# thelovelab/DESeq2

Measured on AMD Instinct MI355X. Metric: genes/sec for DESeq() disp+beta+Wald fit, 50k x 500 x p=4 (throughput of steps pipelined two deep; one call at a time: one_call_at_a_time), higher is better.
Workload: dtype f64; 1 GPU; BASELINE configs[2]: 50k genes x 500 samples, ~batch+condition (p=4), Wald; 50000 non-zero genes in total, sharded over 1 GPU(s) in the contiguous ranges of R/parallel.R:10; inputs resident in HBM in R layout (int32 counts, f64 nf matrix; the fused chain reads the size factors as the m-vector the matrix was built from); genes_total=50000, genes_this_gpu=50000, samples=500, p=4, test=Wald, parallelism=gene-shard x1, chain=fused device-driven (dsq_deseq_dev), steps_overlap=step k enqueued while step k-1's results are copied and post-processed

## Files before the change

deseq2_amd/csrc/aux.hip:

```cpp
#include "dsq_internal.hpp"
#include "dsq_math.hpp"
#include "dsq_wave.hpp"

namespace dsq {

static constexpr int kAuxBatch = 4;

static inline int aux_grid_fwd(int n) {
    int blocks = (n + 3) / 4;
    int cap = device_cu_count() * 8;
    return blocks < cap ? (blocks < 1 ? 1 : blocks) : cap;
}

static constexpr int kTileS = 256;
__host__ __device__ static inline bool aux_tiled(int m, int p) { return (size_t)m * p >= 8192 && p <= 24; }

template <int P, bool USE_W, bool TILED>
__global__ void __launch_bounds__(256) prefit_kernel(PrefitKernelParams kp) {
    extern __shared__ __attribute__((aligned(16))) double tile[];
    const int lane = threadIdx.x & 63;
    const int wave = threadIdx.x >> 6;
    const int waves = blockDim.x >> 6;
    const int m = kp.m;
    double rr[P][P];
// ... 114 lines not shown
#pragma unroll
        for (int c = P - 1; c >= 0; c--) {
            double v = tu[P + c];
#pragma unroll
            for (int k = c + 1; k < P; k++) v = __builtin_fma(-rr[c][k], b[k], v);
            b[c] = v / rr[c][c];
        }
        if (lane == 0 && active) {
            kp.baseMean[g] = mean;
            kp.baseVar[g] = av / (double)(m - 1);
            kp.allZero[g] = (a2[1] == 0.0) ? 1 : 0;
            kp.roughDisp[g] = __builtin_fmax(ae / (double)(m - P), 0.0);
#pragma unroll
            for (int c = 0; c < P; c++) kp.beta_init[(size_t)g + (size_t)kp.n * c] = b[c];
        }
    }
}

template <int P, bool TILED>
__global__ void __launch_bounds__(256) linear_mu_kernel(PrefitKernelParams kp, double mu_floor, double *mu_out) {
    extern __shared__ __attribute__((aligned(16))) double tile[];
    const int lane = threadIdx.x & 63;
    const int wave = threadIdx.x >> 6;
    const int waves = blockDim.x >> 6;
    const int m = kp.m;
    const int nwork = DSQ_NWORK(kp);
    for (int wbase = blockIdx.x * waves; wbase < nwork; wbase += gridDim.x * waves) {
        const int wi = wbase + wave;
        const bool active = wi < nwork;
        if (!TILED && !active) break;
// ... 488 lines not shown
```

deseq2_amd/csrc/ctx.hip:

```cpp
#include "../../include/deseq2_mi355x.h"
#include "dsq_internal.hpp"

#include <cstdarg>
#include <cstdio>
#include <cstdlib>
#include <cstring>
#include <map>
#include <memory>
#include <mutex>
#include <vector>

namespace dsq {

thread_local char g_err[512] = "";
std::mutex g_mu;

int capi_fail(int code, const char *fmt, ...) {
    va_list ap;
    va_start(ap, fmt);
    vsnprintf(g_err, sizeof g_err, fmt, ap);
    va_end(ap);
    return code;
}

int env_int(const char *name, int dflt) {
    const char *v = getenv(name);
    return (v && *v) ? atoi(v) : dflt;
}

const Tuning &tuning() {
    static Tuning t = {env_int("DSQ_BETA_WAVES", 4), env_int("DSQ_BETA_STAGE", -1), env_int("DSQ_BETA_BPC", 0),
                       env_int("DSQ_BETA_LDS_KB", 160),
                       env_int("DSQ_DISP_WAVES", 4), env_int("DSQ_DISP_STAGE", -1), env_int("DSQ_DISP_BPC", 0),
                       env_int("DSQ_DISP_LDS_KB", 160), env_int("DSQ_ABLATE", 0), env_int("DSQ_FORCE_ITERS", 0),
                       env_int("DSQ_DISP_XLDS", 1), env_int("DSQ_BETA_XLDS", 1), env_int("DSQ_DYNAMIC", 1),
                       env_int("DSQ_BETA_CELLS", 1), env_int("DSQ_DISP_CELL_MINP", DSQ_DISP_CELL_MINP),
                       env_int("DSQ_OVERLAP", 1), env_int("DSQ_LPT", 1),
                       env_int("DSQ_LPT_MAXN", 16384), env_int("DSQ_LPT_KEY1", 1), env_int("DSQ_LPT_KEYD", 1), env_int("DSQ_LPT_KEYM", 2),
                       env_int("DSQ_LPT_KEY2", 1), env_int("DSQ_OUTLIER_FIRST", 1)};
    return t;
}

int device_cu_count() {
    static int cached[kMaxDevices];
    int dev = 0;
    if (hipGetDevice(&dev) != hipSuccess || dev < 0 || dev >= kMaxDevices) return 256;
    if (cached[dev] == 0) {
        int v = 0;
        if (hipDeviceGetAttribute(&v, hipDeviceAttributeMultiprocessorCount, dev) != hipSuccess || v <= 0) v = 256;
        cached[dev] = v;
    }
    return cached[dev];
}

// ... 202 lines not shown
```

deseq2_amd/csrc/dsq_internal.hpp:

```cpp
#pragma once
#include <hip/hip_runtime.h>
#include <stdint.h>
#include <functional>
#include <mutex>
#include <string.h>

namespace dsq {

struct DispKernelParams {
    int n, m, p;
    long ld;
    const int32_t *y;
    const double *mu_hat;
    const double *weights;
    const double *x;
    const double *log_alpha_in;
    const double *prior_mean;
    double prior_sigmasq, min_log_alpha, kappa_0, tol, weightThreshold;
    int maxit, usePrior, useWeights, useCR;
    double *log_alpha;
    int32_t *iter, *iter_accept;
    double *last_change, *initial_lp, *initial_dlp, *last_lp, *last_dlp, *last_d2lp;
    const double *grid;
    int ngrid;
// ... 43 lines not shown
};

struct PrefitKernelParams {
    int n, m, p;
    long ld;
    const int32_t *y;
    const double *nf;
    int nf_is_vector;
    const double *weights;
    int useWeights;
    const double *q, *a, *r;
    double *baseMean, *baseVar, *roughDisp, *beta_init;
    int32_t *allZero;
    const int32_t *rows;
    const int32_t *n_dev;
};

struct LogLikeKernelParams {
    int n, m;
    long ld;
    const int32_t *y;
    const double *mu;
    const double *disp;
    const double *weights;
    int useWeights;
    double *loglike;
    const int32_t *rows;
    const int32_t *n_dev;
    const int32_t *skip;
    const double *kconst;
// ... 61 lines not shown
struct ReplaceKernelParams {
    int n, m;
    long ld;
    const int32_t *y;
    const double *nf;
    int nf_is_vector;
    const double *cooks;
    double cutoff, trim;
    const int32_t *replaceable;
    int sortcap;
    int32_t *newCounts, *replace;
    const int32_t *rows;
    const int32_t *n_dev;
    const int32_t *skip;
    int rows_few, beside;
};

struct SizeFactorKernelParams {
    int n, m;
    const void *y;
    long y_si, y_sj;
    const double *nm;
    long nm_si, nm_sj;
    const double *geoMeans;
    const int32_t *control;
    int type;
    int stabilize;
    double *sf;
    double *lgm_out;
    double *nf_out;
// ... 171 lines not shown
    int beta_waves, beta_stage, beta_bpc, beta_lds_kb;
    int disp_waves, disp_stage, disp_bpc, disp_lds_kb;
    int ablate, force_iters;
    int disp_xlds, beta_xlds;
    int dynamic;
    int beta_cells;
    int disp_cell_minp;
    int overlap;
    int lpt;
    int lpt_maxn;
    int lpt_key1;
    int lpt_keyd;
    int lpt_keym;
    int lpt_key2;
    int outlier_first;
};
const Tuning &tuning();

hipError_t launch_transpose_r_to_gm_f64(const double *src, double *dst, int n, int m, long ld, hipStream_t st);
hipError_t launch_transpose_r_to_gm_i32(const int32_t *src, int32_t *dst, int n, int m, long ld, hipStream_t st);
hipError_t launch_counts_f64_to_gm_i32(const double *src, int32_t *dst, int n, int m, long ld, int32_t *bad, hipStream_t st);
hipError_t launch_transpose_gm_to_r_f64(const double *src, double *dst, int n, int m, long ld, hipStream_t st);
hipError_t launch_transpose_gm_to_r_i32(const int32_t *src, int32_t *dst, int n, int m, long ld, hipStream_t st);
hipError_t launch_test_math(int op, const double *a, const double *b, const double *c, double *out, long n, hipStream_t st);

constexpr int kMaxDevices = 64;
int device_cu_count();
#define DSQ_CACHE_PER_DEVICE(a, b)                                                        \
    do {                                                                                  \
        static thread_local int cache_dev_ = -1;                                          \
// ... 48 lines not shown
```

deseq2_amd/csrc/fit_disp.hip:

```cpp
#ifndef DSQ_DISP_WIDE_MIN
#define DSQ_DISP_WIDE_MIN 11
#endif
#define DSQ_WIDE_MIN DSQ_DISP_WIDE_MIN
#include "dsq_internal.hpp"
#include <cstdio>
#include <cstdlib>
#include "dsq_math.hpp"
#include "dsq_rows.hpp"
#include "dsq_wave.hpp"

namespace dsq {

#ifndef DSQ_DISP_LANE_MIN
#define DSQ_DISP_LANE_MIN 4
#endif
#ifndef DSQ_DISP_TRIP_BATCH
#define DSQ_DISP_TRIP_BATCH 4
#endif
#include "../../include/dsq_arith_spec.h"
#ifndef DSQ_DISP_ROWPASS_MIN
#define DSQ_DISP_ROWPASS_MIN DSQ_SPEC_SERIAL_GRAM_MINP
#endif
typedef double DsqMat1[1][DSQ_P][DSQ_P];
typedef double DsqMat2[2][DSQ_P][DSQ_P];
// ... 845 lines not shown
#define DSQ_DISP_MINW_LONG (DSQ_P <= 10 ? 3 : 1)
#endif
template <bool USE_W, bool STAGE, int MODE>
__host__ __device__ constexpr bool disp_global_dv() { return !STAGE && !USE_W && MODE != 2; }
__host__ __device__ inline size_t disp_hist_doubles(int p, int m) { return (p >= 4 && m >= 256 && m <= 2560) ? ((size_t)m + 1) / 2 : 0; }

template <int P, bool USE_W, bool STAGE, int MODE>
__global__ void __launch_bounds__(256, (disp_global_dv<USE_W, STAGE, MODE>() ? DSQ_DISP_MINW_LONG : DSQ_DISP_MINW)) fit_disp_kernel(DispKernelParams kp) {
    extern __shared__ __attribute__((aligned(16))) double smem[];
    const int lane = threadIdx.x & 63;
    const int wave = threadIdx.x >> 6;
    const int waves = blockDim.x >> 6;
    const int m = kp.m;
    const int nwork = DSQ_NWORK(kp);
    if (blockIdx.x * waves >= nwork) return;

    const double *xs = smem;
    const bool serial_gram = disp_serial_gram(P, kp.ncell, m);
    const size_t slab_d = disp_global_dv<USE_W, STAGE, MODE>() ? disp_hist_doubles(P, m) + (serial_gram ? (size_t)3 * m : 0)
                                                               : disp_slab_doubles<USE_W>(m, STAGE, serial_gram);
    const size_t xoff = (STAGE && kp.xlds) ? (size_t)P * m : 0;
    double *slab = smem + xoff + (size_t)wave * slab_d;
    double *arena = smem + xoff + (size_t)waves * slab_d + (size_t)wave * disp_arena_doubles(P, kp.ncell);
    int32_t *cstart_s = reinterpret_cast<int32_t *>(smem + xoff + (size_t)waves * (slab_d + disp_arena_doubles(P, kp.ncell)));
    int32_t *cperm_s = cstart_s + DSQ_CMAX + 2;
    int32_t *crep_s = cperm_s;
    uint8_t *cid_s = reinterpret_cast<uint8_t *>(crep_s + DSQ_CMAX);
    const int C = kp.ncell;
    const bool sorted = disp_sorted<USE_W>(STAGE, C);
    if (C > 0) {
// ... 327 lines not shown
```

deseq2_amd/csrc/outlier.hip:

```cpp
#include "dsq_internal.hpp"
#include "dsq_math.hpp"
#include "dsq_wave.hpp"
#include <type_traits>

namespace dsq {

DSQ_DEV void wave_sort(double *b, int n2, int lane) {
    wave_lds_sync();
    for (int k = 2; k <= n2; k <<= 1) {
        for (int j = k >> 1; j > 0; j >>= 1) {
            for (int t = lane; t < (n2 >> 1); t += 64) {
                int lo = ((t & ~(j - 1)) << 1) | (t & (j - 1));
                int hi = lo | j;
                bool asc = (lo & k) == 0;
                double a = b[lo], c = b[hi];
                if ((a > c) == asc) { b[lo] = c; b[hi] = a; }
            }
            wave_lds_sync();
        }
    }
}

DSQ_DEV void wave_merge_bitonic(double *b, int n2, int lane) {
    wave_lds_sync();
// ... 192 lines not shown
        any = __any(any);
        int32_t *og = kp.newCounts + (size_t)g * kp.ld;
        if (!any) {
            int32_t yb[kOutlierBatch];
            sweep_batched<kOutlierBatch>(m, lane, [&](int j, int b) { yb[b] = yg[j]; }, [&](int j, int b) { og[j] = yb[b]; });
        } else {
            wave_lds_sync();
            for (int k = lane; k < n2; k += 64) buf[k] = k < m ? (double)yg[k] / nfg[k] : inf;
            wave_sort(buf, n2, lane);
            const double tbm = trimmed_mean_sorted(buf, m, kp.trim, lane);
            for (int j = lane; j < m; j += 64) {
                int rep = (int)(tbm * nfg[j]);
                og[j] = (ckg[j] > kp.cutoff && kp.replaceable[j]) ? rep : yg[j];
            }
        }
        if (lane == 0) kp.replace[g] = any ? 1 : 0;
    }
}

static int outlier_waves(size_t doubles_per_wave) {
    const size_t cap = 160 * 1024;
    int w = 4;
    while (w > 0 && (size_t)w * doubles_per_wave * 8 > cap) w >>= 1;
    return w;
}

template <typename KP, typename F>
static hipError_t launch_outlier(F fn, const KP &kp, size_t doubles_per_wave, hipStream_t st, bool *ok) {
    int waves = outlier_waves(doubles_per_wave);
    *ok = waves > 0;
    if (!*ok) return hipSuccess;
// ... 41 lines not shown
```

deseq2_amd/csrc/pipeline.hip:

```cpp
#include "capi.hpp"
#include "dsq_math.hpp"
#include "dsq_wave.hpp"

#include <algorithm>
#include <cstdio>
#include <cstdlib>
#include <cstring>
#include <vector>

namespace dsq {

DSQ_DEV double np_min(double a, double b) { return (a != a || b != b) ? a + b : (a < b ? a : b); }
DSQ_DEV double np_max(double a, double b) { return (a != a || b != b) ? a + b : (a > b ? a : b); }

struct Rows {
    const int32_t *rows;
    const int32_t *n_dev;
    int n;
};
DSQ_DEV int rows_count(const Rows &r) { return r.n_dev ? *r.n_dev : r.n; }
DSQ_DEV int rows_gene(const Rows &r, int i) { return r.rows ? r.rows[i] : i; }

__global__ void __launch_bounds__(1024) compact_kernel(int mode, int n, int32_t *allZero, const int32_t *force_zero,
                                                       const double *mean_in, const double *disp_in, double thresh,
// ... 101 lines not shown
    int32_t *grid_flag, *grid_rows, *grid_count;
    const double *scalars;
    double *dispFit, *log_dfit, *la_init, *dispMAP, *dispersion;
    const double *dispFit_in;
    int32_t *dispIter, *dispOutlier;
    const double *beta_nat, *beta_var, *beta_iter, *logLike;
    double *beta, *betaSE, *stat, *pvalue, *betaIter_out;
    int32_t *betaConv, *optim_flag, *optim_count;
    int32_t *optim_rows;
    int wald;
    const double *beta_init;
    double *opt_start;
    const int32_t *opt_conv;
    LptKey lpt;
    int *lpt_bins;
};

__global__ void alpha_init_kernel(RuleParams q) {
    const int i = blockIdx.x * blockDim.x + threadIdx.x;
    const bool on = i < rows_count(q.rw);
    const int g = on ? rows_gene(q.rw, i) : 0;
    if (on) {
        const double bm = q.baseMean[g], bv = q.baseVar[g];
        const double xim = q.xim_dev ? *q.xim_dev : q.xim;
        const double mom = (bv - xim * bm) / (bm * bm);
        double a = np_min(q.roughDisp[g], mom);
        a = np_min(np_max(q.minDisp, a), q.maxDisp);
        q.alpha_init[g] = a;
        q.la0[g] = dlog(a);
    }
// ... 4 lines not shown
    const int i = blockIdx.x * blockDim.x + threadIdx.x;
    if (i >= rows_count(q.rw)) return;
    const int g = rows_gene(q.rw, i);
    double d = np_min(dexp(q.la_out[g]), q.maxDisp);
    const double ilp = q.initial_lp[g];
    if (q.last_lp[g] < ilp + __builtin_fabs(ilp) / 1e6) d = q.alpha_init[g];
    const int it = q.iter[g];
    q.dispGeneIter[g] = it;
    const bool conv = (it < q.maxit) && !(it == 1);
    const bool refit = !conv && (d > q.minDisp * 10.0);
    q.dge[g] = d;
    q.grid_flag[g] = refit ? 1 : 0;
    if (refit) q.grid_rows[atomicAdd(q.grid_count, 1)] = g;
}

__global__ void gene_est_final_kernel(RuleParams q) {
    const int i = blockIdx.x * blockDim.x + threadIdx.x;
    if (i >= rows_count(q.rw)) return;
    const int g = rows_gene(q.rw, i);
    double d = q.dge[g];
    if (q.grid_flag[g]) d = dexp(q.la_grid[g]);
    q.dge[g] = np_min(np_max(d, q.minDisp), q.maxDisp);
}

__global__ void map_init_kernel(RuleParams q) {
    const int i = blockIdx.x * blockDim.x + threadIdx.x;
    const bool on = i < rows_count(q.rw);
    const int g = on ? rows_gene(q.rw, i) : 0;
    if (on) {
        const double fit = q.dispFit_in ? q.dispFit_in[g] : q.scalars[DSQ_SC_COEF0] + q.scalars[DSQ_SC_COEF1] / q.baseMean[g];
        const double d = q.dge[g];
        double init = (d > 0.1 * fit) ? d : fit;
        if (init != init) init = fit;
        q.dispFit[g] = fit;
        q.log_dfit[g] = dlog(fit);
        q.la_init[g] = dlog(init);
    }
    if (q.lpt.kind != LPT_NONE) lpt_block_hist(on ? lpt_bin(q.lpt, g) : -1, q.lpt_bins);
}

__global__ void map_post_kernel(RuleParams q) {
    const int i = blockIdx.x * blockDim.x + threadIdx.x;
    if (i >= rows_count(q.rw)) return;
    const int g = rows_gene(q.rw, i);
// ... 66 lines not shown
__global__ void optim_post_kernel(RuleParams q) {
    const int cnt = rows_count(q.rw);
    for (int i = blockIdx.x * blockDim.x + threadIdx.x; i < cnt; i += gridDim.x * blockDim.x) {
        const int g = rows_gene(q.rw, i);
        if (q.betaConv && q.opt_conv[g]) q.betaConv[g] = 1;
        if (q.wald && q.stat) {
            for (int c = 0; c < q.p; c++) {
                const double z = q.beta[(size_t)g + (size_t)q.n * c] / q.betaSE[(size_t)g + (size_t)q.n * c];
                q.stat[(size_t)g + (size_t)q.n * c] = z;
                q.pvalue[(size_t)g + (size_t)q.n * c] = dpnorm_upper2(z);
            }
        }
    }
}

__global__ void list_kernel(Rows rw, const int32_t *flag, int want, int32_t *rows_out, int32_t *count) {
    const int i = blockIdx.x * blockDim.x + threadIdx.x;
    if (i >= rows_count(rw)) return;
    const int g = rows_gene(rw, i);
    if ((flag[g] != 0) == (want != 0)) rows_out[atomicAdd(count, 1)] = g;
}

__global__ void cand_list_kernel(Rows rw, const int32_t *bound_flag, const int32_t *optim_flag, int32_t *flag_out, int32_t *rows_out,
                                 int32_t *count) {
    const int i = blockIdx.x * blockDim.x + threadIdx.x;
    if (i >= rows_count(rw)) return;
    const int g = rows_gene(rw, i);
    const int f = (bound_flag[g] != 0 || optim_flag[g] != 0) ? 1 : 0;
    flag_out[g] = f;
    if (f) rows_out[atomicAdd(count, 1)] = g;
}

struct NaRowsParams {
    Rows rw;
    int n, p;
    const int32_t *allZero, *n_refit;
    double *beta, *betaSE, *stat, *pvalue, *betaIter, *logLike, *logLikeReduced, *maxCooks;
    int32_t *betaConv;
};
__global__ void na_rows_kernel(NaRowsParams q) {
    const int i = blockIdx.x * blockDim.x + threadIdx.x;
    if (i >= rows_count(q.rw) || *q.n_refit <= 0) return;
    const int g = rows_gene(q.rw, i);
    if (!q.allZero[g]) return;
    const double nan = dnan();
    for (int c = 0; c < q.p; c++) {
        q.beta[(size_t)g + (size_t)q.n * c] = nan;
        q.betaSE[(size_t)g + (size_t)q.n * c] = nan;
        if (q.stat) { q.stat[(size_t)g + (size_t)q.n * c] = nan; q.pvalue[(size_t)g + (size_t)q.n * c] = nan; }
    }
    q.betaIter[g] = nan; q.logLike[g] = nan; q.maxCooks[g] = nan;
    if (q.logLikeReduced) q.logLikeReduced[g] = nan;
    q.betaConv[g] = -1;
}

__global__ void __launch_bounds__(256) na_assay_rows_kernel(int n, int m, long ld, const int32_t *allZero, double *a0, double *a1,
                                                            int32_t *zero_p = nullptr, int zero_n = 0) {
    if (blockIdx.x == 0 && (int)threadIdx.x < zero_n) zero_p[threadIdx.x] = 0;
    const int lane = threadIdx.x & 63;
    const int g = blockIdx.x * blockDim.x + threadIdx.x;
    unsigned long long todo = __ballot(g < n && allZero[g] != 0);
    const int base = g - lane;
    const double nan = dnan();
    while (todo) {
        const int l = __builtin_ctzll(todo);
        todo &= todo - 1;
        const size_t row = (size_t)(base + l) * ld;
        for (int j = lane; j < m; j += 64) {
            if (a0) a0[row + j] = nan;
            if (a1) a1[row + j] = nan;
        }
    }
}

__global__ void __launch_bounds__(256) masked_max_kernel(Rows rw, int m, long ld, const double *cooks, const int32_t *use,
                                                         const int32_t *zero, int all_replaceable, int valid,
                                                         const int32_t *n_refit, double *maxCooks) {
    if (*n_refit <= 0) return;
    const int lane = threadIdx.x & 63, wave = threadIdx.x >> 6, waves = blockDim.x >> 6;
    const int nw = rows_count(rw);
    for (int wi = blockIdx.x * waves + wave; wi < nw; wi += gridDim.x * waves) {
        const int g = rows_gene(rw, wi);
        if (all_replaceable || !valid) {
            if (lane == 0) maxCooks[g] = dnan();
            continue;
        }
        const double *ck = cooks + (size_t)g * ld;
        double mx = -__builtin_inf();
        int isnan_ = 0;
        for (int j = lane; j < m; j += 64) {
            if (!use[j]) continue;
            double v = zero[j] ? 0.0 : ck[j];
            if (v != v) isnan_ = 1;
// ... 102 lines not shown
    int red_ncell;
    int32_t *cells_dev;
    void *trend_ws, *sel_ws;
    int pkp, pmax;
    int next_counter;
    const int32_t *cell_perm, *cell_start;
    int ncell;
    const char *tag;
    double t_tol, t_minmu, ge_floor;
    int t_maxit, t_useQR;
    hipStream_t side;
    hipEvent_t ev_fork, ev_join;
    bool overlap, forked, ll_pending;
    LogLikeKernelParams ll;
    bool outlier_first, cand_ready, ll_event;
    int any3, maxcell, all_replaceable;
};

enum { CNT_NZ = DSQ_ST_N_NONZERO, CNT_GRID1 = DSQ_ST_N_GRID_GENEEST, CNT_TREND = DSQ_ST_N_TREND, CNT_GRID2 = DSQ_ST_N_GRID_MAP,
       CNT_OPT1 = DSQ_ST_N_OPTIM_GENEEST, CNT_OPT2 = DSQ_ST_N_OPTIM_TEST, CNT_REP = DSQ_ST_N_REPLACE, CNT_REFIT = DSQ_ST_N_REFIT,
       CNT_GRID1R = DSQ_ST_N_GRID_GENEEST_REFIT, CNT_GRID2R = DSQ_ST_N_GRID_MAP_REFIT, CNT_OPT1R = DSQ_ST_N_OPTIM_GENEEST_REFIT,
       CNT_OPT2R = DSQ_ST_N_OPTIM_TEST_REFIT, CNT_OPT3 = 14, CNT_OPT3R = 15, CNT_N = DSQ_ST_COUNT };
static_assert(DSQ_ST_N_OPTIM_TEST_REFIT < 14 && DSQ_ST_COUNT == 16, "status block layout");

static int *next_work_counter(Pipe &P) {
    int *c = P.work_counters + (P.next_counter % 60);
    P.next_counter++;
    return c;
}

static inline dim3 ew_grid(int n) { return dim3((unsigned)((n + 255) / 256 > 0 ? (n + 255) / 256 : 1)); }

static inline int rows_few(const Pipe &P, const Rows &rw) {
    return (rw.rows && rw.rows != P.rows_nz && rw.rows != P.rows_lpt && rw.rows != P.rows_rev) ? 1 : 0;
}

template <class KP>
static KP fit_head(const Pipe &P, const Rows &rw, const int32_t *y, const double *weights) {
    KP kp;
    memset(&kp, 0, sizeof kp);
    kp.n = P.n; kp.m = P.m; kp.ld = P.ld;
    kp.y = y; kp.nf = P.a->nf; kp.nf_is_vector = P.a->nf_is_vector;
    kp.weights = P.a->useWeights ? weights : nullptr; kp.useWeights = kp.weights ? 1 : 0;
    kp.rows = rw.rows; kp.n_dev = rw.n_dev;
    return kp;
}

static RuleParams rule_params(const Pipe &P, const Rows &rw) {
    RuleParams q;
// ... 108 lines not shown
                                       const double *r, double *beta_init) {
    PrefitKernelParams kp = fit_head<PrefitKernelParams>(P, rw, y, nullptr);
    kp.p = p; kp.q = q; kp.a = xr; kp.r = r;
    kp.baseMean = P.cnum; kp.baseVar = P.cden; kp.roughDisp = P.dev; kp.allZero = P.opt_conv; kp.beta_init = beta_init;
    return kp;
}
static LogLikeKernelParams loglike_params(const Pipe &P, const Rows &rw, const int32_t *y, const double *mu, double *out) {
    LogLikeKernelParams lk;
    memset(&lk, 0, sizeof lk);
    lk.n = P.n; lk.m = P.m; lk.ld = P.ld; lk.y = y; lk.mu = mu; lk.disp = P.o->dispersion;
    lk.weights = P.a->useWeights ? P.a->weights_norm : nullptr; lk.useWeights = P.a->useWeights ? 1 : 0;
    lk.loglike = out; lk.rows = rw.rows; lk.n_dev = rw.n_dev; lk.kconst = P.kconst;
    return lk;
}

static int launch_prefit_rows(Pipe &P, const Rows &rw, const int32_t *y) {
    PrefitKernelParams kp = prefit_params(P, rw, y, P.a->weights_raw);
    kp.r = P.a->r;
    kp.baseMean = P.o->baseMean; kp.baseVar = P.o->baseVar; kp.roughDisp = P.roughDisp; kp.beta_init = P.beta_init;
    kp.allZero = P.o->allZero;
    bool ok = false;
    capi_prof_begin(rw.rows ? "prefit_moments:refit" : "prefit_moments", P.n, P.st);
    DSQ_HIP(launch_prefit(kp, P.st, &ok));
    capi_prof_end(P.st);
    if (!ok) return capi_fail(DSQ_ERR_UNSUPPORTED, "dsq_deseq_dev: p=%d", P.p);
    return DSQ_OK;
}

__global__ void copy_rows_cols_kernel(Rows rw, int n, int p, const double *src_a, const double *src_b, double *dst_a, double *dst_b) {
    const int cnt = rows_count(rw);
    for (int i = blockIdx.x * blockDim.x + threadIdx.x; i < cnt; i += gridDim.x * blockDim.x) {
        const int g = rows_gene(rw, i);
        for (int c = 0; c < p; c++) {
// ... 69 lines not shown
    std::sort(b.begin(), b.end());
    if (a != b) return capi_fail(DSQ_ERR_DEVICE, "launch order of %s (key: %s): the list is no permutation of the %d rows", launch, key, cnt);
    fprintf(stderr, "[dsq] launch order: %s by %s, %d rows, permutation ok\n", launch, key, cnt);
    return DSQ_OK;
}
static int lpt_scatter(Pipe &P, const Rows &rw, const RuleParams &q, int32_t *rev) {
    capi_prof_begin("lpt_order", P.n, P.st);
    hipLaunchKernelGGL(lpt_scatter_kernel, ew_grid(P.n), dim3(256), 0, P.st, rw, q.lpt, (const int *)q.lpt_bins, q.lpt_bins + kLptBins,
                       P.rows_lpt, rev);
    capi_prof_end(P.st);
    DSQ_HIP(hipGetLastError());
    return DSQ_OK;
}

static int gene_est(Pipe &P, const Rows &rw, const int32_t *y, double *mu_hat, int cnt_grid, int cnt_optim,
                    int32_t *optim_flag) {
    const DsqDeseqArgs *a = P.a;
    RuleParams q = rule_params(P, rw);
    const bool ord_beta = lpt_applies(P, rw) && !a->linearMu && tuning().lpt_key1 != 0;
    const bool ord_disp = lpt_applies(P, rw) && (tuning().lpt_keyd == 2 || (tuning().lpt_keyd == 1 && P.m >= 256 && P.m <= 1024 && !a->useWeights));
    if (ord_beta || ord_disp) lpt_arm(P, q, LPT_MEAN_UP);
    hipLaunchKernelGGL(alpha_init_kernel, ew_grid(P.n), dim3(256), 0, P.st, q);
    int rc;
    const bool ordered = q.lpt.kind != LPT_NONE;
    int32_t *rev = (ordered && ord_disp) ? P.rows_grid : nullptr;
    if (ordered && (rc = lpt_scatter(P, rw, q, rev))) return rc;
    const Rows up = {P.rows_lpt, rw.n_dev, rw.n}, down = {rev, rw.n_dev, rw.n};
    q.lpt.kind = LPT_NONE;
    if (a->linearMu) {
        bool ok = false;
        capi_prof_begin("linear_mu", P.n, P.st);
// ... 10 lines not shown
        b.optim_flag = optim_flag; b.optim_count = P.counters + cnt_optim;
        hipLaunchKernelGGL(beta_post_kernel, ew_grid(P.n), dim3(256), 0, P.st, b);
        rc = launch_optim(P, cnt_optim, y, P.alpha_init, a->weights_norm, 0.5, P.ge_floor, P.opt_beta, P.opt_se, P.opt_ll, mu_hat);
        if (rc) return rc;
    }
    if (rev && (rc = lpt_verbose(P, "gene-wise fit_disp", lpt_key_name(LPT_MEAN_DOWN), rw, rev))) return rc;
    P.rows_rev = rev;
    rc = launch_fit_disp(P, rev ? down : rw, y, mu_hat, P.la0, P.la0, false, a->weights_floor, a->useCR != 0, false, "fit_disp");
    P.rows_rev = nullptr;
    if (rc) return rc;
    q.grid_count = P.counters + cnt_grid;
    hipLaunchKernelGGL(gene_est_post_kernel, ew_grid(P.n), dim3(256), 0, P.st, q);
    Rows gr = {P.rows_grid, P.counters + cnt_grid, P.n};
    rc = launch_fit_disp(P, gr, y, mu_hat, P.la0, P.la0, false, a->weights_floor, a->useCR != 0, true, "fit_disp_grid");
    if (rc) return rc;
    hipLaunchKernelGGL(gene_est_final_kernel, ew_grid(P.n), dim3(256), 0, P.st, q);
    DSQ_HIP(hipGetLastError());
    return DSQ_OK;
}

static int map_est(Pipe &P, const Rows &rw, const int32_t *y, const double *mu_hat, int cnt_grid) {
    const DsqDeseqArgs *a = P.a;
    RuleParams q = rule_params(P, rw);
    const int keym = (lpt_applies(P, rw) && (tuning().lpt_maxn <= 0 || P.n <= tuning().lpt_maxn)) ? tuning().lpt_keym : 0;
    if (keym) lpt_arm(P, q, keym);
    hipLaunchKernelGGL(map_init_kernel, ew_grid(P.n), dim3(256), 0, P.st, q);
    int rc;
    const bool ordered = q.lpt.kind != LPT_NONE;
    if (ordered && ((rc = lpt_scatter(P, rw, q, nullptr)) || (rc = lpt_verbose(P, "MAP fit_disp", lpt_key_name(q.lpt.kind), rw, P.rows_lpt)))) return rc;
    q.lpt.kind = LPT_NONE;
    rc = launch_fit_disp(P, ordered ? Rows{P.rows_lpt, rw.n_dev, rw.n} : rw, y, mu_hat, P.la_init, P.log_dfit, true, a->weights_norm,
                         a->useCR != 0, false, "fit_disp");
    if (rc) return rc;
    q.grid_count = P.counters + cnt_grid;
    hipLaunchKernelGGL(map_post_kernel, ew_grid(P.n), dim3(256), 0, P.st, q);
    Rows gr = {P.rows_grid, P.counters + cnt_grid, P.n};
    rc = launch_fit_disp(P, gr, y, mu_hat, P.la_init, P.log_dfit, true, a->weights_norm, true, true, "fit_disp_grid");
    if (rc) return rc;
    P.lpt_test.kind = LPT_NONE;
    if (lpt_applies(P, rw) && !a->betaPrior && tuning().lpt_key2 != 2) {
        const int kind = tuning().lpt_key2 == 1 ? LPT_MEAN_UP : (a->linearMu ? LPT_NONE : LPT_ITER_F64);
// ... 202 lines not shown
        if (!repl[j]) all_rep = 0;
    }
    void *mv;
    int rc = capi_upload_table(DSQ_WS_PIPE_OUTLIER_META, meta.data(), meta.size() * sizeof(int32_t), st, &mv);
    if (rc) return rc;
    M->dperm = (int32_t *)mv; M->din3 = M->dperm + m; M->drepl = M->din3 + m; M->duse3 = M->drepl + m; M->dstart = M->duse3 + m;
    M->maxcell = maxcell; M->any3 = any3; M->all_rep = all_rep;
    return DSQ_OK;
}

static int outlier_finish(Pipe &P, const Rows &nz, const Rows &rep, const OutlierMeta &M, const int32_t *n_refit) {
    const DsqDeseqOut *o = P.o;
    const int n = P.n, m = P.m, p = P.p;
    NaRowsParams nr;
    memset(&nr, 0, sizeof nr);
    nr.rw = rep; nr.n = n; nr.p = P.a->betaPrior ? P.a->p_prior : p; nr.allZero = o->allZero; nr.n_refit = n_refit;
    nr.beta = o->beta; nr.betaSE = o->betaSE; nr.stat = o->stat; nr.pvalue = o->pvalue; nr.betaIter = o->betaIter;
    nr.logLike = o->logLike; nr.logLikeReduced = o->logLikeReduced; nr.maxCooks = o->maxCooks; nr.betaConv = o->betaConv;
    hipLaunchKernelGGL(na_rows_kernel, ew_grid(n), dim3(256), 0, P.st, nr);
    int grid = (n + 3) / 4, capg = device_cu_count() * 8;
    if (grid > capg) grid = capg;
    hipLaunchKernelGGL(masked_max_kernel, dim3(grid), dim3(256), 0, P.st, nz, m, P.ld, (const double *)o->cooks,
                       (const int32_t *)M.duse3, (const int32_t *)M.drepl, M.all_rep, (m > p && M.any3) ? 1 : 0, n_refit,
                       o->maxCooks);
    DSQ_HIP(hipGetLastError());
    return DSQ_OK;
}

static size_t align8(size_t v) { return (v + 7) & ~(size_t)7; }

struct WsWalk {
    double *D;
    size_t d = 0, i = 0;
    void operator()(double *&f, size_t k) { if (D) f = D + d; d += align8(k); }
    void operator()(int32_t *&f, size_t k) { if (D) f = (int32_t *)(D + d) + i; i += align8(k); }
    size_t bytes() const { return d * sizeof(double) + i * sizeof(int32_t) + 256; }
};
static size_t workspace_table(Pipe &P, int n, int p, int nt, double *base) {
    const size_t nd = align8((size_t)n), np_ = align8((size_t)n * p), ntd = align8((size_t)nt);
// ... 269 lines not shown
}

static CooksKernelParams cooks_params(const Pipe &P, const OutlierMeta &M, const Rows &rw) {
    const DsqDeseqArgs *a = P.a;
    const DsqDeseqOut *o = P.o;
    CooksKernelParams ck;
    memset(&ck, 0, sizeof ck);
    ck.n = P.n; ck.m = P.m; ck.p = P.p; ck.ld = P.ld; ck.y = a->y; ck.nf = a->nf; ck.nf_is_vector = a->nf_is_vector;
    ck.mu = o->mu; ck.H = o->H; ck.perm = M.dperm; ck.cell_start = M.dstart; ck.in3 = M.din3; ck.ncell = a->ncell; ck.any3 = M.any3;
    int cap = 2; while (cap < (M.any3 ? M.maxcell : P.m)) cap <<= 1;
    ck.sortcap = cap;
    ck.cooks = o->cooks; ck.maxCooks = o->maxCooks; ck.robustDisp = P.robustDisp;
    ck.rows = rw.rows; ck.n_dev = rw.n_dev;
    return ck;
}
static ReplaceKernelParams replace_params(const Pipe &P, const OutlierMeta &M, const Rows &rw) {
    const DsqDeseqArgs *a = P.a;
    const DsqDeseqOut *o = P.o;
    ReplaceKernelParams rk;
    memset(&rk, 0, sizeof rk);
    rk.n = P.n; rk.m = P.m; rk.ld = P.ld; rk.y = a->y; rk.nf = a->nf; rk.nf_is_vector = a->nf_is_vector;
    rk.cooks = o->cooks; rk.cutoff = a->cooksCutoff; rk.trim = a->trim; rk.replaceable = M.drepl;
    int cap2 = 2; while (cap2 < P.m) cap2 <<= 1;
    rk.sortcap = cap2;
    rk.newCounts = o->replaceCounts; rk.replace = o->replace;
    rk.rows = rw.rows; rk.n_dev = rw.n_dev;
    return rk;
}
static int launch_cooks_rows(Pipe &P, const CooksKernelParams &ck, hipStream_t st) {
    bool ok = true;
    capi_prof_begin("cooks_distance", P.n, st);
    DSQ_HIP(launch_cooks(ck, st, &ok));
    capi_prof_end(st);
    if (!ok) return capi_fail(DSQ_ERR_UNSUPPORTED, "m=%d samples: a gene row plus its sort buffer exceeds the 160 KiB LDS", P.m);
    return DSQ_OK;
}
static int launch_replace_rows(Pipe &P, const ReplaceKernelParams &rk, hipStream_t st) {
    bool ok = true;
    capi_prof_begin("replace_outliers", P.n, st);
    DSQ_HIP(launch_replace(rk, st, &ok));
    capi_prof_end(st);
    if (!ok) return capi_fail(DSQ_ERR_UNSUPPORTED, "m=%d samples: the sort buffer exceeds the 160 KiB LDS", P.m);
    return DSQ_OK;
}

static int list_replaced(Pipe &P, const Rows &from) {
    const DsqDeseqOut *o = P.o;
    hipLaunchKernelGGL(list_kernel, ew_grid(P.n), dim3(256), 0, P.st, from, (const int32_t *)o->replace, 1, P.rows_rep, P.counters + CNT_REP);
    const Rows rep = {P.rows_rep, P.counters + CNT_REP, P.n};
    const int rc = launch_prefit_rows(P, rep, o->replaceCounts);
    if (rc) return rc;
    hipLaunchKernelGGL(list_kernel, ew_grid(P.n), dim3(256), 0, P.st, rep, (const int32_t *)o->allZero, 0, P.rows_refit, P.counters + CNT_REFIT);
    return DSQ_OK;
}

static int phase_outlier_detect(Pipe &P, const Rows &nz, const OutlierMeta &M, bool counters_zeroed) {
    const DsqDeseqArgs *a = P.a;
    const DsqDeseqOut *o = P.o;
    const int n = P.n, m = P.m;
    hipStream_t st = P.st;
    if (!counters_zeroed) DSQ_HIP(hipMemsetAsync(P.counters + CNT_REP, 0, (CNT_N - CNT_REP) * sizeof(int32_t), st));
    int rc = launch_cooks_rows(P, cooks_params(P, M, nz), st);
    if (rc) return rc;
    hipLaunchKernelGGL(na_assay_rows_kernel, ew_grid(n), dim3(256), 0, st, n, m, P.ld, (const int32_t *)o->allZero, o->cooks,
                       (double *)nullptr);
    if (!a->do_replace) return DSQ_OK;
    if ((rc = launch_replace_rows(P, replace_params(P, M, nz), st))) return rc;
    return list_replaced(P, nz);
}

static int phase_outlier_refit(Pipe &P, const Rows &nz, const OutlierMeta &M);

static int phase_outlier_first(Pipe &P, const Rows &nz, const OutlierMeta &M, bool counters_zeroed) {
    const DsqDeseqOut *o = P.o;
    const int n = P.n, m = P.m;
    hipStream_t st = P.st;
    if (!counters_zeroed) DSQ_HIP(hipMemsetAsync(P.counters + CNT_REP, 0, (CNT_N - CNT_REP) * sizeof(int32_t), st));
    int32_t *skip = P.rows_lpt, *n_cand = next_work_counter(P);
    if (getenv("DSQ_VERBOSE")) fprintf(stderr, "[dsq] outlier phase: candidates first (n=%d)\n", n);
    hipLaunchKernelGGL(cand_list_kernel, ew_grid(n), dim3(256), 0, st, nz, (const int32_t *)P.grid_flag, (const int32_t *)o->optim_test,
                       skip, P.rows_grid, n_cand);
    hipLaunchKernelGGL(na_assay_rows_kernel, ew_grid(n), dim3(256), 0, st, n, m, P.ld, (const int32_t *)o->allZero, o->cooks,
                       (double *)nullptr);
    int rc;
    if ((rc = fork_side(P)) || (rc = launch_pending_ll(P, true))) return rc;
    DSQ_HIP(hipEventRecord(P.ev_fork, P.side));
    P.ll_event = true;
    CooksKernelParams ck = cooks_params(P, M, nz);
    ReplaceKernelParams rk = replace_params(P, M, nz);
    ck.skip = rk.skip = skip;
    ck.beside = rk.beside = 1;
    if ((rc = launch_cooks_rows(P, ck, P.side)) || (rc = launch_replace_rows(P, rk, P.side))) return rc;
    const Rows cand = {P.rows_grid, n_cand, n};
    ck = cooks_params(P, M, cand); rk = replace_params(P, M, cand);
    ck.rows_few = rk.rows_few = 1;
    if ((rc = launch_cooks_rows(P, ck, st)) || (rc = launch_replace_rows(P, rk, st)) || (rc = list_replaced(P, cand))) return rc;
    return phase_outlier_refit(P, nz, M);
}

static void refit_defaults(Pipe &P) {
    P.tag = ":refit";
    P.t_tol = 1e-8; P.t_maxit = 100; P.t_useQR = 1; P.t_minmu = 0.5; P.ge_floor = 0.5;
}

static int phase_outlier_refit(Pipe &P, const Rows &nz, const OutlierMeta &M) {
    const DsqDeseqArgs *a = P.a;
    const DsqDeseqOut *o = P.o;
    const Rows rep = {P.rows_rep, P.counters + CNT_REP, P.n};
    const Rows rf = {P.rows_refit, P.counters + CNT_REFIT, P.n};
    int rc;
    if ((rc = launch_pending_ll(P, true))) return rc;
    refit_defaults(P);
    if (!a->nf_is_vector) {
        double *b;
        if ((rc = xim_scratch(P, &b))) return rc;
        DSQ_HIP(launch_xim_flagged(a->nf, P.n, P.m, P.ld, o->replace, o->allZero, b, P.xim_dev + 1, P.st));
        P.xim_cur = P.xim_dev + 1;
    }
    if ((rc = gene_est(P, rf, o->replaceCounts, o->mu_hat, CNT_GRID1R, CNT_OPT1R, o->optim_geneest))) return rc;
    if ((rc = map_est(P, rf, o->replaceCounts, o->mu_hat, CNT_GRID2R))) return rc;
    if (P.ll_event) {
        P.ll_event = false;
        DSQ_HIP(hipStreamWaitEvent(P.st, P.ev_fork, 0));
    } else if ((rc = join_side(P))) return rc;
    if ((rc = test_fit(P, rf, o->replaceCounts, o->mu_hat, nullptr, CNT_OPT2R))) return rc;
    if (a->betaPrior && (rc = prior_fit(P, rf, o->replaceCounts, CNT_OPT2R))) return rc;
    if ((rc = join_side(P))) return rc;
    return a->defer_finish ? DSQ_OK : outlier_finish(P, nz, rep, M, P.counters + CNT_REFIT);
}

static int run_chain(const DsqDeseqArgs *a, const DsqDeseqOut *o, hipStream_t st, Pipe &P) {
    int rc = check_args(a, o);
    if (rc || (rc = capi_check_device()) || (rc = bind(P, a, o, st)) || (rc = launch_init_fills(P)) || (rc = prepare_designs(P))) return rc;
    const Rows nz = {P.rows_nz, P.counters + CNT_NZ, P.n};
// ... 46 lines not shown
```

Measured before the change: 5.657 million genes/s.

## Fuse outlier-refit list building and small kernels; raise refit wave priority

The replace and prefit kernels now emit the replaced-gene and refit lists directly through atomic appends, which removes two separate list_kernel passes. The candidate-list and NA-assay kernels merge into one launch, na_rows work moves into masked_max_kernel, and the refit gene_est_final step is deferred and folded into map_init_kernel. Refit-subset dispersion kernels also set a higher wave priority (s_setprio) so the small tail work on the main stream is favoured over the side stream. Together this cuts several small launches on the critical refit path. In exchange, list ordering becomes nondeterministic, and the new priority could slow concurrent side-stream work.

```diff
diff --git a/deseq2_amd/csrc/aux.hip b/deseq2_amd/csrc/aux.hip
--- a/deseq2_amd/csrc/aux.hip
+++ b/deseq2_amd/csrc/aux.hip
@@ -152,6 +152,7 @@
 #pragma unroll
             for (int c = 0; c < P; c++) kp.beta_init[(size_t)g + (size_t)kp.n * c] = b[c];
         }
+        if (kp.list_out && lane == 0 && active && a2[1] != 0.0) kp.list_out[atomicAdd(kp.list_count, 1)] = g;
     }
 }
 
diff --git a/deseq2_amd/csrc/ctx.hip b/deseq2_amd/csrc/ctx.hip
--- a/deseq2_amd/csrc/ctx.hip
+++ b/deseq2_amd/csrc/ctx.hip
@@ -37,7 +37,7 @@
                        env_int("DSQ_BETA_CELLS", 1), env_int("DSQ_DISP_CELL_MINP", DSQ_DISP_CELL_MINP),
                        env_int("DSQ_OVERLAP", 1), env_int("DSQ_LPT", 1),
                        env_int("DSQ_LPT_MAXN", 16384), env_int("DSQ_LPT_KEY1", 1), env_int("DSQ_LPT_KEYD", 1), env_int("DSQ_LPT_KEYM", 2),
-                       env_int("DSQ_LPT_KEY2", 1), env_int("DSQ_OUTLIER_FIRST", 1)};
+                       env_int("DSQ_LPT_KEY2", 1), env_int("DSQ_OUTLIER_FIRST", 1), env_int("DSQ_REFIT_PRIO", 1)};
     return t;
 }
 
diff --git a/deseq2_amd/csrc/dsq_internal.hpp b/deseq2_amd/csrc/dsq_internal.hpp
--- a/deseq2_amd/csrc/dsq_internal.hpp
+++ b/deseq2_amd/csrc/dsq_internal.hpp
@@ -81,6 +81,7 @@
     int32_t *allZero;
     const int32_t *rows;
     const int32_t *n_dev;
+    int32_t *list_out, *list_count;
 };
 
 struct LogLikeKernelParams {
@@ -172,6 +173,7 @@
     const int32_t *n_dev;
     const int32_t *skip;
     int rows_few, beside;
+    int32_t *list_out, *list_count;
 };
 
 struct SizeFactorKernelParams {
@@ -373,6 +375,7 @@
     int lpt_keym;
     int lpt_key2;
     int outlier_first;
+    int refit_prio;
 };
 const Tuning &tuning();
 
diff --git a/deseq2_amd/csrc/fit_disp.hip b/deseq2_amd/csrc/fit_disp.hip
--- a/deseq2_amd/csrc/fit_disp.hip
+++ b/deseq2_amd/csrc/fit_disp.hip
@@ -883,6 +883,7 @@
     const int m = kp.m;
     const int nwork = DSQ_NWORK(kp);
     if (blockIdx.x * waves >= nwork) return;
+    if (kp.rows_few > 1) __builtin_amdgcn_s_setprio(3);
 
     const double *xs = smem;
     const bool serial_gram = disp_serial_gram(P, kp.ncell, m);
diff --git a/deseq2_amd/csrc/outlier.hip b/deseq2_amd/csrc/outlier.hip
--- a/deseq2_amd/csrc/outlier.hip
+++ b/deseq2_amd/csrc/outlier.hip
@@ -230,7 +230,10 @@
                 og[j] = (ckg[j] > kp.cutoff && kp.replaceable[j]) ? rep : yg[j];
             }
         }
-        if (lane == 0) kp.replace[g] = any ? 1 : 0;
+        if (lane == 0) {
+            kp.replace[g] = any ? 1 : 0;
+            if (any && kp.list_out) kp.list_out[atomicAdd(kp.list_count, 1)] = g;
+        }
     }
 }
 
diff --git a/deseq2_amd/csrc/pipeline.hip b/deseq2_amd/csrc/pipeline.hip
--- a/deseq2_amd/csrc/pipeline.hip
+++ b/deseq2_amd/csrc/pipeline.hip
@@ -139,6 +139,7 @@
     const int32_t *opt_conv;
     LptKey lpt;
     int *lpt_bins;
+    int with_gene_final;
 };
 
 __global__ void alpha_init_kernel(RuleParams q) {
@@ -173,13 +174,15 @@
     if (refit) q.grid_rows[atomicAdd(q.grid_count, 1)] = g;
 }
 
+DSQ_DEV void gene_est_final_rule(const RuleParams &q, int g) {
+    double d = q.dge[g];
+    if (q.grid_flag[g]) d = dexp(q.la_grid[g]);
+    q.dge[g] = np_min(np_max(d, q.minDisp), q.maxDisp);
+}
 __global__ void gene_est_final_kernel(RuleParams q) {
     const int i = blockIdx.x * blockDim.x + threadIdx.x;
     if (i >= rows_count(q.rw)) return;
-    const int g = rows_gene(q.rw, i);
-    double d = q.dge[g];
-    if (q.grid_flag[g]) d = dexp(q.la_grid[g]);
-    q.dge[g] = np_min(np_max(d, q.minDisp), q.maxDisp);
+    gene_est_final_rule(q, rows_gene(q.rw, i));
 }
 
 __global__ void map_init_kernel(RuleParams q) {
@@ -187,6 +190,7 @@
     const bool on = i < rows_count(q.rw);
     const int g = on ? rows_gene(q.rw, i) : 0;
     if (on) {
+        if (q.with_gene_final) gene_est_final_rule(q, g);
         const double fit = q.dispFit_in ? q.dispFit_in[g] : q.scalars[DSQ_SC_COEF0] + q.scalars[DSQ_SC_COEF1] / q.baseMean[g];
         const double d = q.dge[g];
         double init = (d > 0.1 * fit) ? d : fit;
@@ -283,15 +287,8 @@
     }
 }
 
-__global__ void list_kernel(Rows rw, const int32_t *flag, int want, int32_t *rows_out, int32_t *count) {
-    const int i = blockIdx.x * blockDim.x + threadIdx.x;
-    if (i >= rows_count(rw)) return;
-    const int g = rows_gene(rw, i);
-    if ((flag[g] != 0) == (want != 0)) rows_out[atomicAdd(count, 1)] = g;
-}
-
-__global__ void cand_list_kernel(Rows rw, const int32_t *bound_flag, const int32_t *optim_flag, int32_t *flag_out, int32_t *rows_out,
-                                 int32_t *count) {
+DSQ_DEV void cand_list_rule(const Rows &rw, const int32_t *bound_flag, const int32_t *optim_flag, int32_t *flag_out, int32_t *rows_out,
+                            int32_t *count) {
     const int i = blockIdx.x * blockDim.x + threadIdx.x;
     if (i >= rows_count(rw)) return;
     const int g = rows_gene(rw, i);
@@ -303,14 +300,11 @@
 struct NaRowsParams {
     Rows rw;
     int n, p;
-    const int32_t *allZero, *n_refit;
-    double *beta, *betaSE, *stat, *pvalue, *betaIter, *logLike, *logLikeReduced, *maxCooks;
+    const int32_t *allZero;
+    double *beta, *betaSE, *stat, *pvalue, *betaIter, *logLike, *logLikeReduced;
     int32_t *betaConv;
 };
-__global__ void na_rows_kernel(NaRowsParams q) {
-    const int i = blockIdx.x * blockDim.x + threadIdx.x;
-    if (i >= rows_count(q.rw) || *q.n_refit <= 0) return;
-    const int g = rows_gene(q.rw, i);
+DSQ_DEV void na_rows_rule(const NaRowsParams &q, int g) {
     if (!q.allZero[g]) return;
     const double nan = dnan();
     for (int c = 0; c < q.p; c++) {
@@ -318,14 +312,12 @@
         q.betaSE[(size_t)g + (size_t)q.n * c] = nan;
         if (q.stat) { q.stat[(size_t)g + (size_t)q.n * c] = nan; q.pvalue[(size_t)g + (size_t)q.n * c] = nan; }
     }
-    q.betaIter[g] = nan; q.logLike[g] = nan; q.maxCooks[g] = nan;
+    q.betaIter[g] = nan; q.logLike[g] = nan;
     if (q.logLikeReduced) q.logLikeReduced[g] = nan;
     q.betaConv[g] = -1;
 }
 
-__global__ void __launch_bounds__(256) na_assay_rows_kernel(int n, int m, long ld, const int32_t *allZero, double *a0, double *a1,
-                                                            int32_t *zero_p = nullptr, int zero_n = 0) {
-    if (blockIdx.x == 0 && (int)threadIdx.x < zero_n) zero_p[threadIdx.x] = 0;
+DSQ_DEV void na_assay_rows_rule(int n, int m, long ld, const int32_t *allZero, double *a0, double *a1) {
     const int lane = threadIdx.x & 63;
     const int g = blockIdx.x * blockDim.x + threadIdx.x;
     unsigned long long todo = __ballot(g < n && allZero[g] != 0);
@@ -341,11 +333,24 @@
         }
     }
 }
+__global__ void __launch_bounds__(256) na_assay_rows_kernel(int n, int m, long ld, const int32_t *allZero, double *a0, double *a1,
+                                                            int32_t *zero_p = nullptr, int zero_n = 0) {
+    if (blockIdx.x == 0 && (int)threadIdx.x < zero_n) zero_p[threadIdx.x] = 0;
+    na_assay_rows_rule(n, m, ld, allZero, a0, a1);
+}
+__global__ void __launch_bounds__(256) cand_front_kernel(Rows rw, const int32_t *bound_flag, const int32_t *optim_flag, int32_t *flag_out,
+                                                         int32_t *rows_out, int32_t *count, int n, int m, long ld, const int32_t *allZero,
+                                                         double *cooks) {
+    cand_list_rule(rw, bound_flag, optim_flag, flag_out, rows_out, count);
+    na_assay_rows_rule(n, m, ld, allZero, cooks, nullptr);
+}
 
 __global__ void __launch_bounds__(256) masked_max_kernel(Rows rw, int m, long ld, const double *cooks, const int32_t *use,
                                                          const int32_t *zero, int all_replaceable, int valid,
-                                                         const int32_t *n_refit, double *maxCooks) {
+                                                         const int32_t *n_refit, double *maxCooks, NaRowsParams na) {
     if (*n_refit <= 0) return;
+    for (int i = blockIdx.x * blockDim.x + threadIdx.x, cnt = rows_count(na.rw); i < cnt; i += gridDim.x * blockDim.x)
+        na_rows_rule(na, rows_gene(na.rw, i));
     const int lane = threadIdx.x & 63, wave = threadIdx.x >> 6, waves = blockDim.x >> 6;
     const int nw = rows_count(rw);
     for (int wi = blockIdx.x * waves + wave; wi < nw; wi += gridDim.x * waves) {
@@ -478,6 +483,7 @@
     bool overlap, forked, ll_pending;
     LogLikeKernelParams ll;
     bool outlier_first, cand_ready, ll_event;
+    bool gene_final_pending;
     int any3, maxcell, all_replaceable;
 };
 
@@ -496,7 +502,7 @@
 static inline dim3 ew_grid(int n) { return dim3((unsigned)((n + 255) / 256 > 0 ? (n + 255) / 256 : 1)); }
 
 static inline int rows_few(const Pipe &P, const Rows &rw) {
-    return (rw.rows && rw.rows != P.rows_nz && rw.rows != P.rows_lpt && rw.rows != P.rows_rev) ? 1 : 0;
+    return (rw.rows && rw.rows != P.rows_nz && rw.rows != P.rows_lpt && rw.rows != P.rows_rev) ? (tuning().refit_prio ? 2 : 1) : 0;
 }
 
 template <class KP>
@@ -635,9 +641,10 @@
     return lk;
 }
 
-static int launch_prefit_rows(Pipe &P, const Rows &rw, const int32_t *y) {
+static int launch_prefit_rows(Pipe &P, const Rows &rw, const int32_t *y, int32_t *list_nonzero = nullptr, int32_t *list_count = nullptr) {
     PrefitKernelParams kp = prefit_params(P, rw, y, P.a->weights_raw);
     kp.r = P.a->r;
+    kp.list_out = list_nonzero; kp.list_count = list_count;
     kp.baseMean = P.o->baseMean; kp.baseVar = P.o->baseVar; kp.roughDisp = P.roughDisp; kp.beta_init = P.beta_init;
     kp.allZero = P.o->allZero;
     bool ok = false;
@@ -737,7 +744,7 @@
 }
 
 static int gene_est(Pipe &P, const Rows &rw, const int32_t *y, double *mu_hat, int cnt_grid, int cnt_optim,
-                    int32_t *optim_flag) {
+                    int32_t *optim_flag, bool defer_final = false) {
     const DsqDeseqArgs *a = P.a;
     RuleParams q = rule_params(P, rw);
     const bool ord_beta = lpt_applies(P, rw) && !a->linearMu && tuning().lpt_key1 != 0;
@@ -778,7 +785,8 @@
     Rows gr = {P.rows_grid, P.counters + cnt_grid, P.n};
     rc = launch_fit_disp(P, gr, y, mu_hat, P.la0, P.la0, false, a->weights_floor, a->useCR != 0, true, "fit_disp_grid");
     if (rc) return rc;
-    hipLaunchKernelGGL(gene_est_final_kernel, ew_grid(P.n), dim3(256), 0, P.st, q);
+    if (defer_final) P.gene_final_pending = true;
+    else hipLaunchKernelGGL(gene_est_final_kernel, ew_grid(P.n), dim3(256), 0, P.st, q);
     DSQ_HIP(hipGetLastError());
     return DSQ_OK;
 }
@@ -788,7 +796,10 @@
     RuleParams q = rule_params(P, rw);
     const int keym = (lpt_applies(P, rw) && (tuning().lpt_maxn <= 0 || P.n <= tuning().lpt_maxn)) ? tuning().lpt_keym : 0;
     if (keym) lpt_arm(P, q, keym);
+    q.with_gene_final = P.gene_final_pending ? 1 : 0;
+    P.gene_final_pending = false;
     hipLaunchKernelGGL(map_init_kernel, ew_grid(P.n), dim3(256), 0, P.st, q);
+    q.with_gene_final = 0;
     int rc;
     const bool ordered = q.lpt.kind != LPT_NONE;
     if (ordered && ((rc = lpt_scatter(P, rw, q, nullptr)) || (rc = lpt_verbose(P, "MAP fit_disp", lpt_key_name(q.lpt.kind), rw, P.rows_lpt)))) return rc;
@@ -1021,15 +1032,14 @@
     const int n = P.n, m = P.m, p = P.p;
     NaRowsParams nr;
     memset(&nr, 0, sizeof nr);
-    nr.rw = rep; nr.n = n; nr.p = P.a->betaPrior ? P.a->p_prior : p; nr.allZero = o->allZero; nr.n_refit = n_refit;
+    nr.rw = rep; nr.n = n; nr.p = P.a->betaPrior ? P.a->p_prior : p; nr.allZero = o->allZero;
     nr.beta = o->beta; nr.betaSE = o->betaSE; nr.stat = o->stat; nr.pvalue = o->pvalue; nr.betaIter = o->betaIter;
-    nr.logLike = o->logLike; nr.logLikeReduced = o->logLikeReduced; nr.maxCooks = o->maxCooks; nr.betaConv = o->betaConv;
-    hipLaunchKernelGGL(na_rows_kernel, ew_grid(n), dim3(256), 0, P.st, nr);
+    nr.logLike = o->logLike; nr.logLikeReduced = o->logLikeReduced; nr.betaConv = o->betaConv;
     int grid = (n + 3) / 4, capg = device_cu_count() * 8;
     if (grid > capg) grid = capg;
     hipLaunchKernelGGL(masked_max_kernel, dim3(grid), dim3(256), 0, P.st, nz, m, P.ld, (const double *)o->cooks,
                        (const int32_t *)M.duse3, (const int32_t *)M.drepl, M.all_rep, (m > p && M.any3) ? 1 : 0, n_refit,
-                       o->maxCooks);
+                       o->maxCooks, nr);
     DSQ_HIP(hipGetLastError());
     return DSQ_OK;
 }
@@ -1329,7 +1339,7 @@
     ck.rows = rw.rows; ck.n_dev = rw.n_dev;
     return ck;
 }
-static ReplaceKernelParams replace_params(const Pipe &P, const OutlierMeta &M, const Rows &rw) {
+static ReplaceKernelParams replace_params(const Pipe &P, const OutlierMeta &M, const Rows &rw, bool list) {
     const DsqDeseqArgs *a = P.a;
     const DsqDeseqOut *o = P.o;
     ReplaceKernelParams rk;
@@ -1340,6 +1350,7 @@
     rk.sortcap = cap2;
     rk.newCounts = o->replaceCounts; rk.replace = o->replace;
     rk.rows = rw.rows; rk.n_dev = rw.n_dev;
+    if (list) { rk.list_out = P.rows_rep; rk.list_count = P.counters + CNT_REP; }
     return rk;
 }
 static int launch_cooks_rows(Pipe &P, const CooksKernelParams &ck, hipStream_t st) {
@@ -1359,14 +1370,9 @@
     return DSQ_OK;
 }
 
-static int list_replaced(Pipe &P, const Rows &from) {
-    const DsqDeseqOut *o = P.o;
-    hipLaunchKernelGGL(list_kernel, ew_grid(P.n), dim3(256), 0, P.st, from, (const int32_t *)o->replace, 1, P.rows_rep, P.counters + CNT_REP);
+static int moments_replaced(Pipe &P) {
     const Rows rep = {P.rows_rep, P.counters + CNT_REP, P.n};
-    const int rc = launch_prefit_rows(P, rep, o->replaceCounts);
-    if (rc) return rc;
-    hipLaunchKernelGGL(list_kernel, ew_grid(P.n), dim3(256), 0, P.st, rep, (const int32_t *)o->allZero, 0, P.rows_refit, P.counters + CNT_REFIT);
-    return DSQ_OK;
+    return launch_prefit_rows(P, rep, P.o->replaceCounts, P.rows_refit, P.counters + CNT_REFIT);
 }
 
 static int phase_outlier_detect(Pipe &P, const Rows &nz, const OutlierMeta &M, bool counters_zeroed) {
@@ -1380,8 +1386,8 @@
     hipLaunchKernelGGL(na_assay_rows_kernel, ew_grid(n), dim3(256), 0, st, n, m, P.ld, (const int32_t *)o->allZero, o->cooks,
                        (double *)nullptr);
     if (!a->do_replace) return DSQ_OK;
-    if ((rc = launch_replace_rows(P, replace_params(P, M, nz), st))) return rc;
-    return list_replaced(P, nz);
+    if ((rc = launch_replace_rows(P, replace_params(P, M, nz, true), st))) return rc;
+    return moments_replaced(P);
 }
 
 static int phase_outlier_refit(Pipe &P, const Rows &nz, const OutlierMeta &M);
@@ -1393,23 +1399,21 @@
     if (!counters_zeroed) DSQ_HIP(hipMemsetAsync(P.counters + CNT_REP, 0, (CNT_N - CNT_REP) * sizeof(int32_t), st));
     int32_t *skip = P.rows_lpt, *n_cand = next_work_counter(P);
     if (getenv("DSQ_VERBOSE")) fprintf(stderr, "[dsq] outlier phase: candidates first (n=%d)\n", n);
-    hipLaunchKernelGGL(cand_list_kernel, ew_grid(n), dim3(256), 0, st, nz, (const int32_t *)P.grid_flag, (const int32_t *)o->optim_test,
-                       skip, P.rows_grid, n_cand);
-    hipLaunchKernelGGL(na_assay_rows_kernel, ew_grid(n), dim3(256), 0, st, n, m, P.ld, (const int32_t *)o->allZero, o->cooks,
-                       (double *)nullptr);
+    hipLaunchKernelGGL(cand_front_kernel, ew_grid(n), dim3(256), 0, st, nz, (const int32_t *)P.grid_flag, (const int32_t *)o->optim_test,
+                       skip, P.rows_grid, n_cand, n, m, P.ld, (const int32_t *)o->allZero, o->cooks);
     int rc;
     if ((rc = fork_side(P)) || (rc = launch_pending_ll(P, true))) return rc;
     DSQ_HIP(hipEventRecord(P.ev_fork, P.side));
     P.ll_event = true;
     CooksKernelParams ck = cooks_params(P, M, nz);
-    ReplaceKernelParams rk = replace_params(P, M, nz);
+    ReplaceKernelParams rk = replace_params(P, M, nz, false);
     ck.skip = rk.skip = skip;
     ck.beside = rk.beside = 1;
     if ((rc = launch_cooks_rows(P, ck, P.side)) || (rc = launch_replace_rows(P, rk, P.side))) return rc;
     const Rows cand = {P.rows_grid, n_cand, n};
-    ck = cooks_params(P, M, cand); rk = replace_params(P, M, cand);
+    ck = cooks_params(P, M, cand); rk = replace_params(P, M, cand, true);
     ck.rows_few = rk.rows_few = 1;
-    if ((rc = launch_cooks_rows(P, ck, st)) || (rc = launch_replace_rows(P, rk, st)) || (rc = list_replaced(P, cand))) return rc;
+    if ((rc = launch_cooks_rows(P, ck, st)) || (rc = launch_replace_rows(P, rk, st)) || (rc = moments_replaced(P))) return rc;
     return phase_outlier_refit(P, nz, M);
 }
 
@@ -1432,7 +1436,7 @@
         DSQ_HIP(launch_xim_flagged(a->nf, P.n, P.m, P.ld, o->replace, o->allZero, b, P.xim_dev + 1, P.st));
         P.xim_cur = P.xim_dev + 1;
     }
-    if ((rc = gene_est(P, rf, o->replaceCounts, o->mu_hat, CNT_GRID1R, CNT_OPT1R, o->optim_geneest))) return rc;
+    if ((rc = gene_est(P, rf, o->replaceCounts, o->mu_hat, CNT_GRID1R, CNT_OPT1R, o->optim_geneest, true))) return rc;
     if ((rc = map_est(P, rf, o->replaceCounts, o->mu_hat, CNT_GRID2R))) return rc;
     if (P.ll_event) {
         P.ll_event = false;
```

Result: no change. 5.661 million genes/s (median of 4 runs) (+0.1%).
